# SudeepDasari/visual_foresight

Hardware: AMD Instinct MI355X
Metric: predicted frames/sec (whole node), 200-sample x 13-step x 64x64 CEM (higher is better)
Workload: dtype f32

## Files before the change

visual_foresight_amd/csrc/vf_conv_gsplit.h:

```cpp
#pragma once
#include <hip/hip_runtime.h>
#include "vf_conv_mfma.h"

namespace vf {

__host__ __device__ inline unsigned gs_live_rows(const int img, const int rem, const int yy, const int n_here,
                                                 const int TH, const int TW, const int ty0, const int tx0, const int Hout,
                                                 const int Wout, const int Hin) {
    const int y = ty0 + yy, x = tx0 + rem - yy * TW;
    if (img >= n_here || rem >= TH * TW || y >= Hout || x >= Wout) return 0u;
    unsigned bits = 0u;
    for (int ky = 0; ky < 5; ++ky) bits |= ((unsigned)(y + ky - 2) < (unsigned)Hin ? 1u : 0u) << ky;
    return bits;
}
enum GsRowVariant { GS_ROW_ALL = 0, GS_ROW_FROM1, GS_ROW_TO3, GS_ROW_TO2, GS_ROW_NONE };
__host__ __device__ constexpr int gs_row_variant(const unsigned live4, const int ky) {
    return ky == 0 ? (live4 == 0u ? GS_ROW_NONE : (!(live4 & 1u) ? GS_ROW_FROM1 : GS_ROW_ALL))
                   : (ky == 4 ? (live4 == 0u ? GS_ROW_NONE : (!(live4 & 12u) ? GS_ROW_TO2 : (!(live4 & 8u) ? GS_ROW_TO3 : GS_ROW_ALL)))
                              : GS_ROW_ALL);
}
__host__ __device__ constexpr int gs_row_first(const int v) { return v == GS_ROW_FROM1 ? 1 : 0; }
__host__ __device__ constexpr int gs_row_end(const int v) {
    return v == GS_ROW_NONE ? 0 : (v == GS_ROW_TO3 ? 3 : (v == GS_ROW_TO2 ? 2 : 4));
}
// ... 37 lines not shown
        }
        gbTab[i] = g; gbTab[gbC + i] = b;
    }

    int ab4[MR];
    unsigned live_rows = 0u;
    {
        const int px_per_img = p.TH * p.TW;
        const TileDiv div_rpi(p.RPI), div_tw(p.TW);
#pragma unroll
        for (int m = 0; m < MR; ++m) {
            const int row = m * 32 + n;
            const int img = div_rpi.div(row), rem = row - img * p.RPI;
            const bool ok = img < p.NI && rem < px_per_img;
            const int y = div_tw.div(rem), x = rem - y * p.TW;
            ab4[m] = ((ok ? (img * tile_px + y * LW + x) * KCpad : 0) + kh * 4) >> 2;
            if constexpr (MR == 4) {
                if (p.pad_skip) {
                    const unsigned bits = gs_live_rows(img, rem, y, min(p.NI, p.B - bimg0), p.TH, p.TW, ty0, tx0, p.Hout,
                                                       p.Wout, p.Hin);
#pragma unroll
                    for (int ky = 0; ky < 5; ++ky)
                        if (__builtin_amdgcn_ballot_w64(((bits >> ky) & 1u) != 0u) != 0ull) live_rows |= 1u << (4 * ky + m);
                }
            }
        }
        live_rows = (MR != 4 || !p.pad_skip) ? 0xFFFFFu : (unsigned)__builtin_amdgcn_readfirstlane((int)live_rows);
    }
    f32x16 acc[MR][1];
#pragma unroll
    for (int m = 0; m < MR; ++m)
#pragma unroll
        for (int r = 0; r < 16; ++r) acc[m][0][r] = 0.f;

    const int Ntot = p.ncg * G * 32;
    const int total_chunks = p.seg[0].nchunk + (p.nseg > 1 ? p.seg[1].nchunk : 0);
    const int gtN = total_chunks * 25;
    const unsigned gs_loff = (unsigned)(((kh * Ntot + (cg * G + wave) * 32 + n) * 4) * 4);
    const unsigned gs_wstep_b = (unsigned)(2 * Ntot * 4) * 4u;
    const __amdgpu_buffer_rsrc_t gs_rsrc =
        __builtin_amdgcn_make_buffer_rsrc(const_cast<float *>(p.Wp), 0, 0x7FFFFFFF, 0x00020000);
    f32x4 gsW[4];
    auto gs_loadq = [&](const int q_, const int gt) {
        const unsigned so_ = (unsigned)(min(gt, gtN - 1) * 4 + q_) * gs_wstep_b;
        gsW[q_] = __builtin_bit_cast(f32x4, __builtin_amdgcn_raw_buffer_load_b128(gs_rsrc, gs_loff, so_, 0));
    };
    const int ci0 = p.chunk_begin;
#pragma unroll
    for (int q_ = 0; q_ < 4; ++q_) gs_loadq(q_, ci0 * 25);

    const unsigned magic_px = 0xFFFFFFFFu / (unsigned)tile_px + 1u, magic_lw = 0xFFFFFFFFu / (unsigned)LW + 1u;
    const int q = tid & (q4 - 1), pl = tid >> q4_log2;
    constexpr int ppp = kConvThreads >> q4_log2;
    const int npix = p.NI * tile_px;
    const int y0 = ty0 - 2, x0 = tx0 - 2;
    const int n_here = min(p.NI, p.B - bimg0);
    const bool ni1 = p.NI == 1;
    struct ChunkSrc {
        __amdgpu_buffer_rsrc_t rsrc;
        unsigned cbyte, cstride, img_step;
        int seg, gi;
        bool has_ln, relu;
    };
    auto chunk_src = [&](const int ci) {
        ChunkSrc cs;
        cs.seg = (ci < p.seg[0].nchunk) ? 0 : 1;
// ... 207 lines not shown
```

visual_foresight_amd/csrc/vf_conv_mfma.h:

```cpp
#pragma once
#include <hip/hip_runtime.h>
#include <type_traits>

#ifdef VF_HOST_SELFTEST
#define VF_GLOBAL __device__
#define VF_LAUNCH_BOUNDS(...)
#else
#define VF_GLOBAL __global__
#define VF_LAUNCH_BOUNDS(...) __launch_bounds__(__VA_ARGS__)
#endif

namespace vf {

constexpr int kPollSleep = 16;

#ifdef VF_TILE_STATS
__device__ unsigned long long g_tile_clk[32][8];
#define VF_TS_NOW() (threadIdx.x == 0 ? wall_clock64() : 0ull)
#define VF_TS_ADD(KEY_, SLOT_, DT_) do { if (threadIdx.x == 0) atomicAdd(&g_tile_clk[KEY_][SLOT_], (unsigned long long)(DT_)); } while (0)
#else
#define VF_TS_NOW() 0ull
#define VF_TS_ADD(KEY_, SLOT_, DT_) do { } while (0)
#endif

// ... 78 lines not shown
    int KC;
    int NI, TH, TW, RPI;
    int tilesY, tilesX;
    int ncg;
    int Cout;
    const float *Wp;
    const unsigned short *Wp16;
    const float *bias;
    const float *sbias;
    int sbias_ld;
    float *out;
    float *cstate;
    const float *cstate_in;
    long long cin_bstride;
    long long *stats;
    int stats_nparts;
    int chunks_per_split;
    int n_valid;
    int tile_variant;
    const void *fuse_comp;
    const void *fuse_next;
    int *fuse_ready;
    const int *fuse_status;
    int fuse_view, fuse_nd;
    const int *late_cnt;
    int late_expect, late_mode;
    int *late_status;
    int *cu_state;
    int yield_budget;
    int wt_out;
    const float *cond_bias;
    int chunk_begin;
    int pad_skip;
};

constexpr unsigned kLateSpinLimit = 1u << 26;

constexpr int kYieldSleep = 8;
constexpr int kCtlMyState = 40, kCtlPartnerState = 42;
__device__ __forceinline__ int *ctl_state_word(const int which) {
    extern __shared__ __attribute__((aligned(16))) float smem_all[];
    return *reinterpret_cast<int *const *>(smem_all + which);
}
template <class PT>
__device__ __forceinline__ void cu_publish(const PT &p, const int critical) {
    if (p.cu_state != nullptr && threadIdx.x == 0)
        __hip_atomic_store(ctl_state_word(kCtlMyState), critical, __ATOMIC_RELAXED, __HIP_MEMORY_SCOPE_AGENT);
}
template <class PT>
__device__ __forceinline__ const int *cu_partner_word(const PT &) {
    const unsigned long long a = reinterpret_cast<unsigned long long>(ctl_state_word(kCtlPartnerState));
    const unsigned lo = __builtin_amdgcn_readfirstlane((unsigned)a), hi = __builtin_amdgcn_readfirstlane((unsigned)(a >> 32));
    return reinterpret_cast<const int *>(((unsigned long long)hi << 32) | lo);
}
__device__ __forceinline__ unsigned yield_peek_issue(const int *word) {
    unsigned v;
    asm volatile("s_load_dword %0, %1, 0x0 glc" : "=s"(v) : "s"(word) : "memory");
    return v;
}
__device__ __forceinline__ unsigned yield_peek_wait(unsigned v) {
    asm volatile("s_waitcnt lgkmcnt(0)" : "+s"(v) : : "memory");
    return v;
}
__device__ __forceinline__ void yield_to_partner(const int *word, unsigned seen, int &budget) {
    seen = yield_peek_wait(seen);
    if (seen == 0u || budget <= 0) return;
// ... 369 lines not shown
                __hip_atomic_store(dst + 1, sq, __ATOMIC_RELAXED, __HIP_MEMORY_SCOPE_AGENT);
            } else {
                dst[0] = su; dst[1] = sq;
            }
        };
        if (p.NI == 1) {
            if (tid == 0 && bimg0 < p.B) {
                long long su = 0, sq = 0;
                for (int w = 0; w < 4; ++w) { su += red[2 * w]; sq += red[2 * w + 1]; }
                put(p.stats + ((long long)bimg0 * p.stats_nparts + tile_id * p.ncg + cg) * 2, su, sq);
            }
        } else {
            const int waves_per_img = p.RPI / WROWS;
            if (lane == 0 && (wave % waves_per_img) == 0) {
                const int img = wave / waves_per_img;
                const int b = bimg0 + img;
                if (img < p.NI && b < p.B) {
                    long long su = 0, sq = 0;
                    for (int w = 0; w < waves_per_img; ++w) { su += red[2 * (wave + w)]; sq += red[2 * (wave + w) + 1]; }
                    put(p.stats + ((long long)b * p.stats_nparts + cg) * 2, su, sq);
                }
            }
        }
    }
}

template <class F, int... I>
__device__ __forceinline__ void static_for_impl(F &&f, std::integer_sequence<int, I...>) {
    (f(std::integral_constant<int, I>{}), ...);
}
template <int N, class F>
__device__ __forceinline__ void static_for(F &&f) { static_for_impl(f, std::make_integer_sequence<int, N>{}); }

constexpr int kGsXchFloats = 4 * 4 * 16 * 64;
constexpr int kGsCondFloats = kGsXchFloats + 16 + 25 * 128 + 128;
template <int MR, class PT>
__device__ __forceinline__ void lstm_gsplit_epilogue(const PT &p, f32x16 (&acc)[MR][1], const int bx, const int by,
                                                     float *smem) {
    const int tid = threadIdx.x, lane = tid & 63, wave = tid >> 6;
    const int n = lane & 31, kh = lane >> 5;
    const int cg = by;
    const int tiles_per_img = p.tilesY * p.tilesX;
    int bimg0, ty0, tx0, tile_id;
    if (p.NI == 1) {
        bimg0 = bx / tiles_per_img;
        tile_id = bx % tiles_per_img;
        ty0 = (tile_id / p.tilesX) * p.TH;
        tx0 = (tile_id % p.tilesX) * p.TW;
    } else {
        bimg0 = bx * p.NI;
        tile_id = 0; ty0 = 0; tx0 = 0;
    }
    const int ch = cg * 32 + n;
    float *xch = smem;
    long long *red = reinterpret_cast<long long *>(smem + MR * 4 * 16 * 64);
    const bool wt = p.wt_out != 0;

    const long long img_elems = (long long)p.Hout * p.Wout * p.Cout;
    const TileDiv div_rpi(p.RPI), div_tw(p.TW);
    const int n_here = min(p.NI, p.B - bimg0);
    const unsigned img_bytes = (unsigned)img_elems * 4u;
    const unsigned cin_step = (unsigned)p.cin_bstride * 4u;
    const int span_out = n_here > 0 ? (int)((unsigned)(n_here - 1) * img_bytes + img_bytes) : 0;
    const int span_cin = n_here > 0 ? (int)((unsigned)(n_here - 1) * cin_step + img_bytes) : 0;
    const __amdgpu_buffer_rsrc_t r_cin = __builtin_amdgcn_make_buffer_rsrc(
        const_cast<float *>(p.cstate_in + (long long)bimg0 * p.cin_bstride), 0, span_cin, 0x00020000);
// ... 303 lines not shown
    else if constexpr (EPI == EPI_BIAS_RELU) ts_key = p.KH == 1 ? 17 : (p.seg[0].C == 32 ? 18 : 19);
    else if constexpr (EPI == EPI_CONVT_RELU) ts_key = p.nseg == 1 ? 20 : 21;
    else if constexpr (EPI == EPI_PARTIAL) ts_key = 22;
    else if constexpr (is_top_fused(EPI)) ts_key = 23;
    else if constexpr (EPI == EPI_CONVT_RAW_STATS) ts_key = 24;
    const bool late = p.late_cnt != nullptr;
    ln_table(p, bimg0, lnTab, 0, late ? 1 : 2);
    [[maybe_unused]] const bool yielding = kInLaunch && EPI == EPI_LSTM && (GSPLIT || ROW32) && late &&
                                           p.cu_state != nullptr && p.yield_budget > 0;
    [[maybe_unused]] int ybudget = p.yield_budget;
    [[maybe_unused]] const int *yword = yielding ? cu_partner_word(p) : nullptr;

    const int px_per_img = p.TH * p.TW;
    int abase[MR];
    {
        const TileDiv div_rpi(p.RPI), div_tw(p.TW);
#pragma unroll
        for (int m = 0; m < MR; ++m) {
            const int row = wrow0 + m * 32 + n;
            const int img = div_rpi.div(row), rem = row - img * p.RPI;
            const bool ok = img < p.NI && rem < px_per_img;
            const int y = div_tw.div(rem), x = rem - y * p.TW;
            abase[m] = (ok ? (img * tile_px + y * p.stride * LW + x * p.stride) * KCpad : 0) + kh * 4;
        }
    }

    f32x16 acc[MR][GA];
#pragma unroll
    for (int m = 0; m < MR; ++m)
#pragma unroll
        for (int g = 0; g < GA; ++g)
#pragma unroll
            for (int r = 0; r < 16; ++r) acc[m][g][r] = 0.f;

    const int ntaps = p.KH * p.KW;
    const int Ntot = p.ncg * G * 32;
    const int total_chunks = p.seg[0].nchunk + (p.nseg > 1 ? p.seg[1].nchunk : 0);
    const int ch_begin = bz * p.chunks_per_split;
    const int ch_end = min(ch_begin + p.chunks_per_split, total_chunks);
    const float *wlane = p.Wp + ((long long)kh * Ntot + (cg * G) * 32 + n) * 4;
    const long long wstep = (long long)2 * Ntot * 4;

    const int q4 = KC >> 2;
    const int q4_log2 = 31 - __builtin_clz((unsigned)q4);
    const unsigned magic_px = 0xFFFFFFFFu / (unsigned)tile_px + 1u, magic_lw = 0xFFFFFFFFu / (unsigned)LW + 1u;
    const int items = p.NI * tile_px * q4;

    constexpr bool kGbTab = EPI == EPI_LSTM;
    const int gbC = kGbTab ? ((p.seg[0].C + (p.nseg > 1 ? p.seg[1].C : 0) + 3) & ~3) : 0;
    float *gbTab = lnTab + 4 * p.NI + 16;
    if constexpr (kGbTab) {
        for (int i = tid; i < gbC; i += kConvThreads) {
            const int sgi = i < p.seg[0].C ? 0 : 1;
            const int cc = sgi ? i - p.seg[0].C : i;
            float g = 1.f, b = 0.f;
            if (sgi < p.nseg && cc < p.seg[sgi].C && p.seg[sgi].ln_part) {
                const int m = cc % p.seg[sgi].gamma_mod;
                g = p.seg[sgi].gamma[m]; b = p.seg[sgi].beta[m];
            }
            gbTab[i] = g; gbTab[gbC + i] = b;
        }
    }
    f32x4 *bsm = reinterpret_cast<f32x4 *>(gbTab + 2 * gbC);
    const float *wgate = p.Wp + ((long long)kh * Ntot + (cg * G + (wave & (G - 1))) * 32 + n) * 4;
    const int gt0 = ch_begin * ntaps, gtN = ch_end * ntaps;
    f32x4 breg[4];
#define VF_LOADB(GT_)                                                                           \
    _Pragma("unroll") for (int q = 0; q < 4; ++q)                                               \
        if (q < K8) breg[q] = *reinterpret_cast<const f32x4 *>(wgate + ((long long)(GT_) * K8 + q) * wstep);
#define VF_WRITEB(BUF_)                                                                         \
    _Pragma("unroll") for (int q = 0; q < 4; ++q)                                               \
// ... 562 lines not shown
```

visual_foresight_amd/csrc/vf_engine.hip:

```cpp
#include <hip/hip_runtime.h>

#include <algorithm>
#include <cmath>
#include <cstdio>
#include <cstring>
#include <cstdlib>
#include <string>
#include <vector>

#include <dlfcn.h>
#ifdef VF_HOST_SELFTEST
#include <sys/mman.h>
#endif

#include "../../include/vf_hip.h"
#include "vf_conv_mfma.h"
#include "vf_small_kernels.h"
#include "vf_goal_image.h"
#include "vf_frame_scorer.h"
#include "vf_plan_render.h"
#include "vf_conv_bf16x6.h"
#include "vf_persistent.h"

#ifndef VF_WT_DEFAULT
// ... 315 lines not shown
                                    const size_t unit = ((((size_t)(ci * ntaps + tap) * l.ncg + cgi) * 4 + g) * 3 + pl) * 64 +
                                                        kh * 32 + nn;
                                    out[unit * 8 + j] = pc[pl];
                                }
                            }
    }
    return out;
}

static std::vector<float> pack_bias(const ConvLayer &l, const float *b) {
    const int G = l.G;
    std::vector<float> out((size_t)l.ncg * G * 32, 0.f);
    for (int cgi = 0; cgi < l.ncg; ++cgi)
        for (int g = 0; g < G; ++g)
            for (int nn = 0; nn < 32; ++nn) {
                const int co = cgi * 32 + nn;
                if (co >= l.Cout) continue;
                const int src = l.mode == PACK_LSTM ? g * l.Cout + co : co;
                out[((size_t)cgi * G + g) * 32 + nn] = b[src];
            }
    return out;
}

}

using namespace vf;

struct BatchView {
    float *enc0_o, *enc1_o, *enc2_o, *enc3_o, *enc4_o, *enc5_o, *enc6_o;
    float *enc00_o, *enc7_o;
    float *c_state[7], *h_state[7][2];
    long long *st_enc0, *st_h[7], *st_enc6, *st_enc00, *st_enc7;
    float *sbias, *fc_part, *kern;
    float *cond_bias[7][2];
    float *frames_all, *distrib_all, *states_all;
    double *sums;
    const float *actions;
};

struct LayerW { float *w = nullptr, *b = nullptr; unsigned short *w16 = nullptr; };
struct ViewData {
    LayerW lw[kNumConvLayers];
    float *ln_g[kNumLn] = {nullptr}, *ln_b[kNumLn] = {nullptr};
    float *w_rgb = nullptr, *b_rgb = nullptr, *w_mask = nullptr, *b_mask = nullptr;
    float *w_state = nullptr, *b_state = nullptr, *w_sa = nullptr, *b_fc = nullptr;
    float *w_cond[7] = {nullptr};
    float *ctx_frames = nullptr, *ctx_distrib = nullptr;
};

struct AllocRec { void *p; size_t bytes; };

struct vf_handle {
    vf_config cfg;
    int H, W, T, S, ND, K;
    bool savp = false;
    vf::Savp3 *s3 = nullptr;
    bool cond = false;
    float *cond_bias[7] = {nullptr};
    int Hc, Wc;
    int c_t2 = 64, c_top = 32;
    int ncam = 1, n_draws = 1;
    int ntiles;
    int nblocks;
    std::vector<TensorDesc> table;
    size_t blob_floats = 0;
    bool have_weights = false, have_context = false;
// ... 27 lines not shown
    double *goal_mse = nullptr;

    std::vector<AllocRec> allocs;

    bool dedup = true;
    std::vector<BatchView> shared_views;

    bool persistent = false;
    int n_cu = 256;
    float *actions_buf = nullptr;
    struct SchedCache {
        PhaseDesc *d_phases = nullptr;
        int B = -1, items = 0, counters = 0, phases = 0;
        bool dedup = true;
        int xcd_queues = 0, nq = 1, total_q[kQueues] = {0};
        int options = -1;
        double flops = 0.0;
        size_t lds = 0;
        std::vector<int> types, nitems;
    } sched[2];
    int last_sched = 0;
    size_t sched_capacity = 0, counter_capacity = 0;
    PhaseDesc *stage[kSchedRing] = {nullptr};
    hipEvent_t stage_done[kSchedRing] = {nullptr};
    bool stage_used[kSchedRing] = {false};
    int stage_next = 0;
    int *d_sync = nullptr;
    int xcd_queues = kQueues;
    bool early_start = true;
    bool fuse_top = true;
    bool fuse_pair = true;
    bool wt_publish = VF_WT_DEFAULT != 0;
    bool pad_skip = true;
    int yield_budget = -1;
    bool pair_allowed = true;
    int *d_status = nullptr;
    unsigned long long *d_stats = nullptr;
    bool phase_stats = false;
    int persist_wgs_per_cu = 2;
    size_t max_lds = 0;

    bool cache_shared = true, shared_valid = false;
    int shared_cfg = -1;

    bool profiling = false;
    std::vector<hipEvent_t> ev_pool;
    size_t ev_used = 0;
    double prof_flops = 0.0;

#ifdef VF_HOST_SELFTEST
    char *fake_base = nullptr;
    size_t fake_used = 0, fake_size = 0;
    unsigned long long upload_checksum = 0;
#endif
};

namespace vf {

template <typename T>
static int dev_alloc(vf_handle *h, T **p, size_t n) {
    const size_t bytes = std::max<size_t>(n, 1) * sizeof(T);
    void *q = nullptr;
#ifdef VF_HOST_SELFTEST
    const size_t aligned = (bytes + 255) & ~(size_t)255;
    if (h->fake_used + aligned > h->fake_size) return fail(VF_ERR_NOMEM, "self-test address space exhausted");
    q = h->fake_base + h->fake_used;
// ... 439 lines not shown
        for (int k = 0; k < 7; ++k) VF_ALLOC(h->cond_bias[k], 2 * BV * kCondClasses * 4 * L[k]);
    VF_ALLOC(h->fc_part, BV * h->fc.nsplit * kTaps * h->K);
    VF_ALLOC(h->kern, BV * kTaps * h->K);
    VF_ALLOC(h->frames_all, BV * h->T * H * W * 3);
    VF_ALLOC(h->distrib_all, BV * h->T * H * W * ND);
    VF_ALLOC(h->states_all, BV * h->T * cfg->sdim);
    h->sums_view_stride = (long long)Bc * ND * h->nblocks * 2;
    h->sums_step_stride = h->sums_view_stride * NV;
    VF_ALLOC(h->sums, (size_t)h->T * h->sums_step_stride);
    VF_ALLOC(h->goal_mse, BV * h->T);
    VF_ALLOC(h->actions_buf, (size_t)Bc * h->T * cfg->adim);
    h->sched_capacity = ((size_t)h->S * 32 + 8) * NV;
    h->counter_capacity = ((size_t)h->S * 32 + 8) * ((size_t)Bc + 1) * NV;
    VF_ALLOC(h->sched[0].d_phases, h->sched_capacity);
    VF_ALLOC(h->sched[1].d_phases, h->sched_capacity);
    VF_ALLOC(h->d_sync, kSyncHead + h->counter_capacity);
    VF_ALLOC(h->d_status, 1);
    VF_ALLOC(h->d_stats, h->sched_capacity * 2);
    for (int i = 0; i < NV; ++i) {
        BatchView sv;
        memset(&sv, 0, sizeof(sv));
        VF_ALLOC(sv.enc0_o, (size_t)H2 * W2 * 32);
        VF_ALLOC(sv.enc1_o, (size_t)H4 * W4 * L[1]);
        VF_ALLOC(sv.enc2_o, (size_t)H8 * W8 * L[3]);
        VF_ALLOC(sv.enc3_o, (size_t)H8 * W8 * L[3]);
        VF_ALLOC(sv.enc4_o, (size_t)H4 * W4 * L[4]);
        VF_ALLOC(sv.enc5_o, (size_t)H2 * W2 * h->c_t2);
        for (int k = 0; k < 7; ++k) {
            const size_t per = (size_t)lh[k] * lw[k] * L[k];
            VF_ALLOC(sv.c_state[k], per);
            VF_ALLOC(sv.h_state[k][0], per);
            VF_ALLOC(sv.h_state[k][1], per);
            VF_ALLOC(sv.st_h[k], (size_t)h->st_rows[k] * 2);
        }
        VF_ALLOC(sv.st_enc0, (size_t)h->enc0.stats_nparts * 2);
        if (h->savp) {
            VF_ALLOC(sv.enc00_o, (size_t)Hc * Wc * kEnc00Ch);
            VF_ALLOC(sv.st_enc00, (size_t)h->enc00.stats_nparts * 2);
        }
        VF_ALLOC(sv.sbias, (size_t)L[3]);
        if (h->cond)
            for (int k = 0; k < 7; ++k) {
                VF_ALLOC(sv.cond_bias[k][0], (size_t)2 * kCondClasses * 4 * L[k]);
                sv.cond_bias[k][1] = sv.cond_bias[k][0] + (size_t)kCondClasses * 4 * L[k];
            }
        h->shared_views.push_back(sv);
    }
#undef VF_ALLOC
    return VF_OK;
}

extern "C" {

int vf_create(const vf_config *cfg, vf_handle **out) {
    vf_handle *made = nullptr;
    VF_API_TRY
    if (!out) return fail(VF_ERR_INVALID, "null out pointer");
    *out = nullptr;
    int rc = validate(cfg);
    if (rc) return rc;
#ifndef VF_HOST_SELFTEST
    VF_HIP_CHECK(hipSetDevice(cfg->device));
#endif
    vf_handle *h = new vf_handle();
    made = h;
    h->cfg = *cfg;
    if (const char *e = getenv("VF_PAD_SKIP")) h->pad_skip = atoi(e) != 0;
    h->ncam = std::max(1, cfg->ncam);
    h->n_draws = std::max(1, cfg->n_draws);
    h->cfg.ncam = h->ncam; h->cfg.n_draws = h->n_draws;
    h->H = cfg->height; h->W = cfg->width; h->ND = cfg->ndesig; h->K = cfg->num_masks;
    h->T = cfg->sequence_length - cfg->n_context;
    h->S = h->T + cfg->n_context - 1;
    h->table = tensor_table(*cfg);
    h->blob_floats = h->table.back().offset + h->table.back().size();
    h->savp = cfg->arch == 1 || cfg->arch == 2;
    h->cond = cfg->arch == 2;
    h->Hc = h->savp ? h->H / 2 : h->H; h->Wc = h->savp ? h->W / 2 : h->W;
    const int H = h->H, W = h->W;
    h->ntiles = ((H + kCompTile - 1) / kCompTile) * ((W + kCompTile - 1) / kCompTile);
    h->nblocks = sum_blocks(H, W);
#ifdef VF_HOST_SELFTEST
    h->fake_size = (size_t)1 << 40;
    void *base = mmap(nullptr, h->fake_size, PROT_NONE, MAP_PRIVATE | MAP_ANONYMOUS | MAP_NORESERVE, -1, 0);
    if (base == MAP_FAILED) { delete h; return fail(VF_ERR_NOMEM, "self-test address reservation failed"); }
    h->fake_base = static_cast<char *>(base);
#endif

    rc = cfg->arch == 3 ? s3_create(h) : cdna_create(h);
    if (rc) { vf_destroy(h); return rc; }
    VF_INJECT(3);
#ifndef VF_HOST_SELFTEST
    if (hipMemset(h->d_sync, 0, kSyncHead * sizeof(int)) != hipSuccess || hipMemset(h->d_status, 0, sizeof(int)) != hipSuccess) {
        vf_destroy(h);
        return fail(VF_ERR_HIP, "hipMemset of the scheduler words failed");
    }
    for (int i = 0; i < kSchedRing; ++i) {
        void *q = nullptr;
        if (hipHostMalloc(&q, h->sched_capacity * sizeof(PhaseDesc), hipHostMallocDefault) != hipSuccess ||
            hipEventCreateWithFlags(&h->stage_done[i], hipEventDisableTiming) != hipSuccess) {
// ... 208 lines not shown
    v.enc6_o = h->enc6_o + b * Hc * Wc * h->c_top;
    for (int k = 0; k < 7; ++k) {
        const size_t per = (size_t)lh[k] * lw[k] * L[k];
        v.c_state[k] = h->c_state[k] + b * per;
        v.h_state[k][0] = h->h_state[k][0] + b * per;
        v.h_state[k][1] = h->h_state[k][1] + b * per;
        v.st_h[k] = h->st_h[k] + b * h->st_rows[k] * 2;
    }
    v.st_enc0 = h->st_enc0 + b * h->enc0.stats_nparts * 2;
    v.st_enc6 = h->st_enc6 + b * h->convt3.stats_nparts * 2;
    v.sbias = h->sbias + b * L[3];
    if (h->cond)
        for (int k = 0; k < 7; ++k)
            for (int par = 0; par < 2; ++par)
                v.cond_bias[k][par] = h->cond_bias[k] + ((size_t)par * c.max_batch * h->ncam + b) * kCondClasses * 4 * L[k];
    v.fc_part = h->fc_part + b * h->fc.nsplit * kTaps * h->K;
    v.kern = h->kern + b * kTaps * h->K;
    v.frames_all = h->frames_all + b * T * H * W * 3;
    v.distrib_all = h->distrib_all + b * T * H * W * ND;
    v.states_all = h->states_all + b * T * c.sdim;
    v.sums = h->sums + (long long)view * h->sums_view_stride + (size_t)b0 * ND * h->nblocks * 2;
    v.actions = d_actions + (size_t)b0 * T * c.adim;
    return v;
}

static const int kSkipped = 1 << 30;

#ifndef VF_HOST_SELFTEST
struct LaunchSink {
    vf_handle *h;
    hipStream_t st;
    static int skipped() { return VF_OK; }

    int conv(int type, const ConvLayer &l, const ConvParams &p, std::initializer_list<int>) {
        switch (type) {
            case PH_LSTM: {
                if (!h->profiling) return launch_lstm(l, p, st);
                while (h->ev_pool.size() < h->ev_used + 2) {
                    hipEvent_t e;
                    VF_HIP_CHECK(hipEventCreate(&e));
                    h->ev_pool.push_back(e);
                }
                VF_HIP_CHECK(hipEventRecord(h->ev_pool[h->ev_used], st));
                int r = launch_lstm(l, p, st);
                VF_HIP_CHECK(hipEventRecord(h->ev_pool[h->ev_used + 1], st));
                h->ev_used += 2;
                h->prof_flops += 2.0 * (p.B * l.Hout * l.Wout * 25.0 - (p.pad_skip ? 5.0 * gs_pad_skipped_pairs(l, p.B) : 0.0)) *
                                 (l.segC[0] + l.segC[1]) * 4.0 * l.Cout;
                return r;
            }
            case PH_CONV_RELU: return launch_conv_t<1, EPI_BIAS_RELU>(l, p, st);
            case PH_CONV_RAW:
                if (l.tile == TILE_FIRST_VALU) {
                    const dim3 grid(p.B * l.tilesY * l.tilesX);
                    if (l.Cout == 16) hipLaunchKernelGGL(conv_first_kernel<16>, grid, dim3(kConvThreads), l.lds_bytes, st, p);
                    else hipLaunchKernelGGL(conv_first_kernel<32>, grid, dim3(kConvThreads), l.lds_bytes, st, p);
                    VF_HIP_CHECK(hipGetLastError());
                    return VF_OK;
                }
                return launch_conv_t<1, EPI_RAW_STATS>(l, p, st);
            case PH_CONVT_RELU: return launch_conv_t<4, EPI_CONVT_RELU>(l, p, st);
            case PH_CONVT_RAW: return launch_conv_t<4, EPI_CONVT_RAW_STATS>(l, p, st);
            case PH_CONV_RAW3: return l.mrep == 2 ? launch_conv_m<1, EPI_RAW, 2>(l, p, st) : launch_conv_m<1, EPI_RAW, 1>(l, p, st);
            case PH_CONV_RAW3G2: return l.mrep == 2 ? launch_conv_m<2, EPI_RAW, 2>(l, p, st) : launch_conv_m<2, EPI_RAW, 1>(l, p, st);
            case PH_CONV_RAW3G4: return launch_conv_m<4, EPI_RAW, 1>(l, p, st);
            case PH_GATES_RAW: {
                const int tiles = l.NI == 1 ? p.B * l.tilesY * l.tilesX : (p.B + l.NI - 1) / l.NI;
                hipLaunchKernelGGL(conv_gates_raw_kernel, dim3(tiles, l.ncg), dim3(kConvThreads), l.lds_bytes, st, p);
                VF_HIP_CHECK(hipGetLastError());
                return VF_OK;
            }
            default: return launch_conv_t<1, EPI_PARTIAL>(l, p, st);
        }
    }
    int ew(const EwParams &p, int , std::initializer_list<int>) {
        const int items = p.spi > 0 ? (p.B + p.spi - 1) / p.spi : p.B * p.gx;
        const size_t lds = ew_lds_bytes(p.op, h->ND);
        switch (h->ND) {
            case 1: hipLaunchKernelGGL(ew_kernel<1>, dim3(items), dim3(kConvThreads), lds, st, p); break;
            case 2: hipLaunchKernelGGL(ew_kernel<2>, dim3(items), dim3(kConvThreads), lds, st, p); break;
            case 3: hipLaunchKernelGGL(ew_kernel<3>, dim3(items), dim3(kConvThreads), lds, st, p); break;
            default: hipLaunchKernelGGL(ew_kernel<4>, dim3(items), dim3(kConvThreads), lds, st, p); break;
        }
        VF_HIP_CHECK(hipGetLastError());
        return VF_OK;
    }
    int lstm(const ConvLayer &l, const ConvParams &p, int , int , int  = -1) { return conv(PH_LSTM, l, p, {}); }
    int cond(const CondParams &p, std::initializer_list<int>) {
        hipLaunchKernelGGL(cond_bias_kernel, dim3((p.B + kCondPerItem - 1) / kCondPerItem), dim3(256), 0, st, p);
        VF_HIP_CHECK(hipGetLastError());
        return VF_OK;
    }
    int conv_late(int type, const ConvLayer &l, const ConvParams &p, int , int , int  = -1) { return conv(type, l, p, {}); }
    static bool pair_capable() { return false; }
    static const ConvLayer &fc_plan(const vf_handle *h) { return h->fc; }
    int conv_pair(const ConvLayer &, const ConvParams &, const ConvLayer &, const ConvParams &, std::initializer_list<int>) {
        return VF_ERR_INVALID;
    }
    int sa(const SaParams &p, std::initializer_list<int>) {
        hipLaunchKernelGGL(sa_kernel, dim3(p.B), dim3(64), 0, st, p);
        return VF_OK;
    }
    int fin(const FinParams &p, std::initializer_list<int>) {
// ... 235 lines not shown
        s.ln_inv_n = (float)(1.0 / (double)count); s.gamma = g; s.beta = b; s.gamma_mod = gmod; s.relu = relu;
        return s;
    };
#define VF_EMIT(var, expr)                 \
    const int var = (expr);                \
    if (Sink::failed(var)) return var;
#define VF_EMIT_SH(var, shared, expr) VF_EMIT(var, ((shared) && skip_shared) ? Sink::skipped() : (expr))

    int last = -1;
    int u_cond_next[7] = {-1, -1, -1, -1, -1, -1, -1};
    int u_prev[7] = {-1, -1, -1, -1, -1, -1, -1};
    for (int s = 0; s < h->S; ++s) {
        const int cur = s & 1, nxt = cur ^ 1;
        const bool produce = s >= nc - 1;
        const int t_out = s - (nc - 1);
        const bool enc0_sh = enc_shared(s), enc_sh = core_shared(s), all_sh = all_shared(s);
        const BatchView &E0 = enc0_sh ? sh : v;
        const BatchView &E = enc_sh ? sh : v;
        const BatchView &D = all_sh ? sh : v;
        const int BE0 = enc0_sh ? 1 : B, BE = enc_sh ? 1 : B, BD = all_sh ? 1 : B;
        auto bs = [](bool shared, long long per) { return shared ? 0LL : per; };

        SaParams sp; memset(&sp, 0, sizeof(sp));
        if (s < nc - 1) { sp.action = h->ctx_actions + (size_t)s * c.adim; sp.action_bstride = 0; }
        else { sp.action = v.actions + (size_t)(s - (nc - 1)) * c.adim; sp.action_bstride = (long long)T * c.adim; }
        if (s < nc) { sp.state = h->ctx_states + (size_t)s * c.sdim; sp.state_bstride = 0; }
        else { sp.state = v.states_all + (size_t)(s - nc) * c.sdim; sp.state_bstride = (long long)T * c.sdim; }
        sp.adim = c.adim; sp.sdim = c.sdim; sp.B = BD;
        sp.w_state = vd.w_state; sp.b_state = vd.b_state; sp.w_sa = vd.w_sa; sp.n_out = L[3];
        sp.state_out = produce ? v.states_all + (size_t)t_out * c.sdim : nullptr;
        sp.state_out_bstride = (long long)T * c.sdim;
        sp.sbias = D.sbias;
        VF_EMIT_SH(u_sa, all_sh, sink.sa(sp, {last}))

        int u_cond[7];
        for (int k = 0; k < 7; ++k) u_cond[k] = u_cond_next[k];
        auto emit_cond = [&](const int sc, const int u_state, int (&out)[7]) -> int {
            for (int k = 0; k < 7; ++k) out[k] = -1;
            if (!h->cond || sc >= h->S) return VF_OK;
            const float *act, *sta; long long act_bs, sta_bs;
            if (sc < nc - 1) { act = h->ctx_actions + (size_t)sc * c.adim; act_bs = 0; }
            else { act = v.actions + (size_t)(sc - (nc - 1)) * c.adim; act_bs = (long long)T * c.adim; }
            if (sc < nc) { sta = h->ctx_states + (size_t)sc * c.sdim; sta_bs = 0; }
            else { sta = v.states_all + (size_t)(sc - nc) * c.sdim; sta_bs = (long long)T * c.sdim; }
            for (int k = 0; k < 7; ++k) {
                const bool shd = lstm_shared(k, sc);
                CondParams cq; memset(&cq, 0, sizeof(cq));
                cq.action = act; cq.action_bstride = act_bs;
                cq.state = sta; cq.state_bstride = sta_bs;
                cq.adim = c.adim; cq.sdim = c.sdim; cq.B = shd ? 1 : B;
                cq.w = vd.w_cond[k]; cq.C4 = 4 * L[k];
                cq.out = (shd ? sh : v).cond_bias[k][sc & 1];
                VF_EMIT_SH(u_ck, shd, sink.cond(cq, {u_state}))
                out[k] = u_ck;
            }
            return VF_OK;
        };
        if (s == 0) {
            const int rc0 = emit_cond(0, -1, u_cond);
            if (Sink::failed(rc0)) return rc0;
        }

        const float *frame_in; long long frame_bs;
        if (s < nc) { frame_in = vd.ctx_frames + (size_t)s * H * W * 3; frame_bs = 0; }
        else { frame_in = v.frames_all + (size_t)(s - nc) * H * W * 3; frame_bs = (long long)T * H * W * 3; }

// ... 8 lines not shown
            enc00_n = normed(E0.enc00_o, bs(enc0_sh, (long long)Hc * Wc * kEnc00Ch), E0.st_enc00, h->enc00.stats_nparts,
                             h->enc00.stats_nparts, enc0_sh, (long long)Hc * Wc * kEnc00Ch, vd.ln_g[9], vd.ln_b[9],
                             kEnc00Ch, 1);
        }
        p = params(h->enc0, BE0, h->savp ? enc00_n : plain(frame_in, frame_bs), nullptr);
        p.out = E0.enc0_o; p.stats = E0.st_enc0;
        VF_EMIT_SH(u_enc0, enc0_sh, sink.conv(PH_CONV_RAW, h->enc0, p, {u_enc00}))

        SegArg enc0_n = normed(E0.enc0_o, bs(enc0_sh, (long long)H2 * W2 * 32), E0.st_enc0, h->enc0.stats_nparts,
                               h->enc0.stats_nparts, enc0_sh, (long long)H2 * W2 * 32, vd.ln_g[0], vd.ln_b[0], 32, 1);
        auto h_normed = [&](int k) {
            const bool shd = lstm_shared(k, s);
            const BatchView &O = shd ? sh : v;
            const long long per = (long long)lh[k] * lw[k] * L[k];
            return normed(O.h_state[k][nxt], bs(shd, per), O.st_h[k], lstm_plan(k, shd ? 1 : B).stats_nparts,
                          h->st_rows[k], shd, per, vd.ln_g[k + 1], vd.ln_b[k + 1], L[k], 0);
        };
        auto lstm_params = [&](int k, const SegArg &x) {
            const bool out_sh = lstm_shared(k, s), in_sh = lstm_shared(k, s - 1);
            const BatchView &O = out_sh ? sh : v, &I = in_sh ? sh : v;
            const long long per = (long long)lh[k] * lw[k] * L[k];
            SegArg hs = plain(I.h_state[k][cur], bs(in_sh, per));
            ConvParams q = params(lstm_plan(k, out_sh ? 1 : B), out_sh ? 1 : B, hs, &x);
            q.out = O.h_state[k][nxt]; q.cstate = O.c_state[k]; q.stats = O.st_h[k];
            q.stats_nparts = h->st_rows[k];
            q.cstate_in = I.c_state[k]; q.cin_bstride = bs(in_sh, per);
            if (h->cond) q.cond_bias = O.cond_bias[k][s & 1];
#ifdef VF_DEBUG_KNOBS
            static const bool no_rec = getenv("VF_TIMING_NO_RECURRENT") && atoi(getenv("VF_TIMING_NO_RECURRENT"));
            if (no_rec) { q.seg[0].nchunk = 0; q.chunks_per_split = q.seg[1].nchunk; }
#endif
            return q;
        };
        VF_EMIT_SH(u_l1, lstm_shared(0, s), sink.lstm(lstm_plan(0, lstm_shared(0, s) ? 1 : B), lstm_params(0, enc0_n), u_prev[0], u_enc0, u_cond[0]))
        VF_EMIT_SH(u_l2, lstm_shared(1, s), sink.lstm(lstm_plan(1, lstm_shared(1, s) ? 1 : B), lstm_params(1, h_normed(0)), u_prev[1], u_l1, u_cond[1]))

        p = params(h->enc1, BE, h_normed(1), nullptr);
        p.out = E.enc1_o;
        VF_EMIT_SH(u_enc1, enc_sh, sink.conv(PH_CONV_RELU, h->enc1, p, {u_l2}))

        VF_EMIT_SH(u_l3, lstm_shared(2, s), sink.lstm(lstm_plan(2, lstm_shared(2, s) ? 1 : B),
                                lstm_params(2, plain(E.enc1_o, bs(enc_sh, (long long)H4 * W4 * L[1]))), u_prev[2], u_enc1, u_cond[2]))
        VF_EMIT_SH(u_l4, lstm_shared(3, s), sink.lstm(lstm_plan(3, lstm_shared(3, s) ? 1 : B), lstm_params(3, h_normed(2)), u_prev[3], u_l3, u_cond[3]))

        const ConvLayer &enc2_l = light_plan(h->enc2, h->enc2_one, BE);
        const ConvLayer &enc3_l = light_plan(h->enc3, h->enc3_one, BD);
        p = params(enc2_l, BE, h_normed(3), nullptr);
        p.out = E.enc2_o;
        ConvParams p3 = params(enc3_l, BD, plain(E.enc2_o, bs(enc_sh, (long long)H8 * W8 * L[3])), nullptr);
        p3.out = D.enc3_o; p3.sbias = D.sbias; p3.sbias_ld = L[3];
        int u_enc3 = -1;
        const bool pair_ok = Sink::pair_capable() && h->fuse_pair && enc_sh == all_sh && BE == BD;
        if (pair_ok && !ScheduleSink::pairable(enc2_l, enc3_l) && ScheduleSink::pairable(enc2_l, h->enc3)) {
            p3 = params(h->enc3, BD, plain(E.enc2_o, bs(enc_sh, (long long)H8 * W8 * L[3])), nullptr);
            p3.out = D.enc3_o; p3.sbias = D.sbias; p3.sbias_ld = L[3];
            VF_EMIT_SH(u_pair, enc_sh, sink.conv_pair(enc2_l, p, h->enc3, p3, {u_l4, u_sa}))
            u_enc3 = u_pair;
        } else if (pair_ok && ScheduleSink::pairable(enc2_l, enc3_l)) {
            VF_EMIT_SH(u_pair, enc_sh, sink.conv_pair(enc2_l, p, enc3_l, p3, {u_l4, u_sa}))
            u_enc3 = u_pair;
        } else {
            VF_EMIT_SH(u_enc2, enc_sh, sink.conv(PH_CONV_RELU, enc2_l, p, {u_l4}))
            VF_EMIT_SH(u_enc3_, all_sh, sink.conv(PH_CONV_RELU, enc3_l, p3, {u_enc2, u_sa}))
            u_enc3 = u_enc3_;
        }

        VF_EMIT_SH(u_l5, lstm_shared(4, s), sink.lstm(lstm_plan(4, lstm_shared(4, s) ? 1 : B),
                                lstm_params(4, plain(D.enc3_o, bs(all_sh, (long long)H8 * W8 * L[3]))), u_prev[4], u_enc3, u_cond[4]))
        SegArg h5n = h_normed(4);

        const ConvLayer &convt1_l = light_plan(h->convt1, h->convt1_one, BD);
        p = params(convt1_l, BD, h5n, nullptr);
        p.out = D.enc4_o;
        {
            const int rcn = emit_cond(s + 1, u_sa, u_cond_next);
            if (Sink::failed(rcn)) return rcn;
        }
        VF_EMIT_SH(u_t1, all_sh, sink.conv(PH_CONVT_RELU, convt1_l, p, {u_l5}))
        VF_EMIT_SH(u_l6, lstm_shared(5, s), sink.lstm(lstm_plan(5, lstm_shared(5, s) ? 1 : B),
                                lstm_params(5, plain(D.enc4_o, bs(all_sh, (long long)H4 * W4 * L[4]))), u_prev[5], u_t1, u_cond[5]))

        int u_fin = -1, u_fc = -1;
        if (produce) {
            SegArg flat = h5n;
            const ConvLayer &fc_l = Sink::fc_plan(h);
            p = params(fc_l, B, flat, nullptr);
            p.out = v.fc_part;
            VF_EMIT(u_fc_, sink.conv(PH_FC_PARTIAL, fc_l, p, {u_l5}))
            u_fc = u_fc_;
        }

        SegArg enc1_s = plain(E.enc1_o, bs(enc_sh, (long long)H4 * W4 * L[1])), h6n = h_normed(5);
        p = params(h->convt2, BD, enc1_s, &h6n);
        p.out = D.enc5_o;
        VF_EMIT_SH(u_t2, all_sh, sink.conv_late(PH_CONVT_RELU, h->convt2, p, u_enc1, u_l6))
        VF_EMIT_SH(u_l7, lstm_shared(6, s), sink.lstm(lstm_plan(6, lstm_shared(6, s) ? 1 : B),
                                lstm_params(6, plain(D.enc5_o, bs(all_sh, (long long)H2 * W2 * h->c_t2))), u_prev[6], u_t2, u_cond[6]))
        last = u_l7;
        {
            const int now[7] = {u_l1, u_l2, u_l3, u_l4, u_l5, u_l6, u_l7};
            for (int k = 0; k < 7; ++k) u_prev[k] = now[k];
        }
        if (produce) {
            FinParams fp;
            fp.partial = v.fc_part; fp.nsplit = h->fc.nsplit; fp.B = B; fp.K = h->K;
            fp.bias = vd.b_fc; fp.kern = v.kern;
            u_fin = sink.fin(fp, {u_fc});
            if (Sink::failed(u_fin)) return u_fin;
        }

        if (produce) {
            SegArg h7n = h_normed(6);
            p = params(h->convt3, B, enc0_n, &h7n);
            p.out = v.enc6_o; p.stats = v.st_enc6;
            const ConvLayer *top_l = &h->convt3;
            int top_early = u_enc0, top_late = u_l7;
            if (h->savp) {
                SegArg enc6_n = normed(v.enc6_o, (long long)Hc * Wc * 32, v.st_enc6, h->convt3.stats_nparts,
                                       h->convt3.stats_nparts, false, (long long)Hc * Wc * 32, vd.ln_g[8], vd.ln_b[8], 32, 1);
                VF_EMIT(u_t3, sink.conv_late(PH_CONVT_RAW, h->convt3, p, u_enc0, u_l7))
                p = params(h->convt4, B, enc00_n, &enc6_n);
                p.out = v.enc7_o; p.stats = v.st_enc7;
                top_l = &h->convt4; top_early = u_enc00; top_late = u_t3;
            }

            CompositeParams cp; memset(&cp, 0, sizeof(cp));
            cp.B = B; cp.H = H; cp.W = W; cp.ND = ND; cp.K = h->K;
            if (h->savp) {
                cp.enc6 = v.enc7_o; cp.ln_part = v.st_enc7; cp.ln_nparts = h->convt4.stats_nparts;
                cp.gamma = vd.ln_g[10]; cp.beta = vd.ln_b[10];
// ... 177 lines not shown
        ticket += P.n_items;
        if (P.ndep < 0 || P.ndep > kMaxDeps) return fail(VF_ERR_INVALID, "bad dependency count");
        for (int d = 0; d < P.ndep; ++d) {
            bool found = false;
            for (size_t j = 0; j < i && !found; ++j) found = bs.phases[j].cnt_base == P.dep[d].cnt_base;
            if (!found) return fail(VF_ERR_INVALID, "phase " + std::to_string(i) + " depends on a later phase");
            if (P.dep[d].expect <= 0) return fail(VF_ERR_INVALID, "non-positive expected count");
        }
        if (P.has_late) {
            bool found = false;
            for (size_t j = 0; j < i && !found; ++j) found = bs.phases[j].cnt_base == P.late.cnt_base;
            if (!found || !(ph_is_conv(P.type) || P.type == PH_TOP_FUSED) || P.late.expect <= 0)
                return fail(VF_ERR_INVALID, "phase " + std::to_string(i) + ": bad late dependency");
        }
        const int ncnt = P.whole ? 1 : (P.type == PH_TOP_FUSED ? 2 * P.B : P.B);
        if (P.cnt_base < 0 || P.cnt_base + ncnt > bs.counters) return fail(VF_ERR_INVALID, "counter out of range");
        bool ok = true;
        if (P.type == PH_CONV_PAIR) {
            const ConvParams &c2 = P.conv2;
            ok = ok && P.conv.ncg == 1 && c2.ncg == 2 && c2.KC == 32 && c2.nseg == 1 && c2.seg[0].nchunk == 2;
            ok = ok && in_allocs(h, c2.Wp, (size_t)2 * 4 * 2 * 64 * 4 * 4) && in_allocs(h, c2.bias, 64 * 4);
            ok = ok && in_allocs(h, c2.out, (size_t)P.B * c2.Hout * c2.Wout * c2.Cout * 4);
            ok = ok && in_allocs(h, c2.sbias, c2.sbias ? (size_t)((P.B - 1) * c2.sbias_ld + c2.Cout) * 4 : 0);
        }
        if (P.type <= PH_FC_PARTIAL || ph_is_conv(P.type) || P.type == PH_TOP_FUSED || P.type == PH_CONV_PAIR) {
            const ConvParams &c = P.conv;
            for (int s = 0; s < c.nseg; ++s) {
                const long long span = (long long)(P.B - 1) * c.seg[s].bstride + (long long)c.Hin * c.Win * c.seg[s].C;
                ok = ok && in_allocs(h, c.seg[s].ptr, (size_t)span * 4);
                ok = ok && in_allocs(h, c.seg[s].ln_part, c.seg[s].ln_part ? (size_t)((P.B - 1) * c.seg[s].ln_bstride + c.seg[s].ln_nparts * 2) * 8 : 0);
            }
            ok = ok && in_allocs(h, c.Wp, 16) && in_allocs(h, c.bias, 4) && in_allocs(h, c.out, 4);
            ok = ok && in_allocs(h, c.cstate, 4) && in_allocs(h, c.cstate_in, 4) && in_allocs(h, c.stats, 8);
        }
        if (P.conv.wt_out != 0) {
            const bool lstm_vec = P.type == PH_LSTM &&
                                  (P.tile == TILE_LSTM_GS128 || P.tile == TILE_LSTM_GS64 || P.tile == TILE_LSTM_ROW32);
            const bool light_vec = P.type >= PH_CONV_RELU && P.type <= PH_CONVT_RAW && P.conv.Cout % 4 == 0 &&
                                   ((P.tile == TILE_CONV && P.mrep == 1) ||
                                    (P.tile == TILE_FIRST_VALU && P.type == PH_CONV_RAW && (P.conv.Cout == 16 || P.conv.Cout == 32)));
            const bool raw3_vec = (P.type == PH_CONV_RAW3 || P.type == PH_CONV_RAW3G2 || P.type == PH_CONV_RAW3G4) &&
                                  P.tile == TILE_CONV && (P.mrep == 1 || P.mrep == 2) && P.conv.Cout % 4 == 0;
            if (!(lstm_vec || light_vec || raw3_vec || P.type == PH_GATES_RAW || P.type == PH_TOP_FUSED))
                return fail(VF_ERR_INVALID, "phase " + std::to_string(i) + ": write-through publish on a tile with plain stores");
        }
        if (P.type == PH_EW && P.ew.wt != 0) {
            const int op = P.ew.op;
            const bool vec = op == EW_INORM || op == EW_INCELL || op == EW_UPSAMPLE ||
                             (op == EW_TOP3 && P.ew.top.H % 4 == 0 && P.ew.top.W % 16 == 0);
            if (!vec) return fail(VF_ERR_INVALID, "phase " + std::to_string(i) + ": write-through publish on an item with plain stores");
        }
        if (P.type == PH_TOP_FUSED && (P.aux_base != P.cnt_base + P.B || P.aux_base + P.B > bs.counters))
            return fail(VF_ERR_INVALID, "fused phase: bad auxiliary counters");
        if (P.type <= PH_FC_PARTIAL || ph_is_conv(P.type)) {
        } else if (P.type == PH_EW) {
            const EwParams &e = P.ew;
            if (e.op == EW_INORM || e.op == EW_INCELL) {
                const NormParams &q = e.norm;
                const size_t hw = (size_t)q.H * q.W, ctot = (size_t)(e.op == EW_INCELL ? 4 : 1) * q.C;
                ok = ok && in_allocs(h, q.in, ((size_t)(P.B - 1) * q.in_bs + hw * ctot) * 4);
                const size_t co = q.split > 0 ? (size_t)q.split : (size_t)q.C;
                ok = ok && in_allocs(h, q.out, ((size_t)(P.B - 1) * q.out_bs + hw * co) * 4);
                ok = ok && (q.split == 0 || (in_allocs(h, q.out2, ((size_t)(P.B - 1) * q.out_bs + hw * co) * 4) && q.C == 2 * q.split));
                ok = ok && in_allocs(h, q.cond, q.cond ? ((size_t)(P.B - 1) * q.cond_bs + 25 * ctot) * 4 : 0);
                ok = ok && in_allocs(h, q.g0, ctot * 4) && in_allocs(h, q.b0, ctot * 4) && q.C % q.cpi == 0 && e.gx == q.C / q.cpi;
                ok = ok && in_allocs(h, q.tab, q.tab ? (size_t)P.B * q.C * 2 * 4 : 0);
// ... 782 lines not shown
```

Before: 42660.

## Share recurrent gate partial sums across samples when hidden state is still shared

When an LSTM layer's previous-step hidden state was shared across all samples (batch-1) but the current step is per-sample, the recurrent half of the gate convolution is computed once for a single image into a scratch buffer. The per-sample LSTM kernels then start their accumulators from that buffer via acc_init and only process the input-channel chunks (chunk_begin offset). This removes redundant recurrent-weight convolution work across the batch. The cost is an extra launch and a dependency edge, plus a scratch buffer and extra per-lane loads at accumulator init.

```diff
diff --git a/visual_foresight_amd/csrc/vf_conv_gsplit.h b/visual_foresight_amd/csrc/vf_conv_gsplit.h
--- a/visual_foresight_amd/csrc/vf_conv_gsplit.h
+++ b/visual_foresight_amd/csrc/vf_conv_gsplit.h
@@ -93,6 +93,9 @@
     for (int m = 0; m < MR; ++m)
 #pragma unroll
         for (int r = 0; r < 16; ++r) acc[m][0][r] = 0.f;
+    if constexpr (!RAW) {
+        if (p.acc_init != nullptr) gs_acc_init<MR>(p, acc, cg, ty0, tx0);
+    }
 
     const int Ntot = p.ncg * G * 32;
     const int total_chunks = p.seg[0].nchunk + (p.nseg > 1 ? p.seg[1].nchunk : 0);
diff --git a/visual_foresight_amd/csrc/vf_conv_mfma.h b/visual_foresight_amd/csrc/vf_conv_mfma.h
--- a/visual_foresight_amd/csrc/vf_conv_mfma.h
+++ b/visual_foresight_amd/csrc/vf_conv_mfma.h
@@ -134,6 +134,7 @@
     const float *cond_bias;
     int chunk_begin;
     int pad_skip;
+    const float *acc_init;
 };
 
 constexpr unsigned kLateSpinLimit = 1u << 26;
@@ -569,6 +570,30 @@
 template <int N, class F>
 __device__ __forceinline__ void static_for(F &&f) { static_for_impl(f, std::make_integer_sequence<int, N>{}); }
 
+template <int MR, class PT>
+__device__ __forceinline__ void gs_acc_init(const PT &p, f32x16 (&acc)[MR][1], const int cg, const int ty0, const int tx0) {
+    const int lane = threadIdx.x & 63, wave = threadIdx.x >> 6;
+    const int n = lane & 31, kh = lane >> 5;
+    const unsigned px_b = (unsigned)(4 * p.Cout) * 4u;
+    const unsigned col_b = (unsigned)(wave * p.Cout + cg * 32 + n) * 4u;
+    const __amdgpu_buffer_rsrc_t rs = __builtin_amdgcn_make_buffer_rsrc(
+        const_cast<float *>(p.acc_init), 0, (int)((unsigned)(p.Hout * p.Wout) * px_b), 0x00020000);
+    const TileDiv div_tw(p.TW);
+#pragma unroll
+    for (int m = 0; m < MR; ++m)
+#pragma unroll
+        for (int j = 0; j < 4; ++j) {
+            const int rem = m * 32 + 8 * j + 4 * kh;
+            const int yy = div_tw.div(rem);
+            const int y = ty0 + yy, x = tx0 + rem - yy * p.TW;
+            const bool ok = rem < p.TH * p.TW && y < p.Hout && x < p.Wout;
+            const unsigned off = (ok ? (unsigned)(y * p.Wout + x) * px_b : 0u) + col_b;
+#pragma unroll
+            for (int i = 0; i < 4; ++i)
+                acc[m][0][4 * j + i] = __builtin_bit_cast(float, __builtin_amdgcn_raw_buffer_load_b32(rs, off, (unsigned)i * px_b, 0));
+        }
+}
+
 constexpr int kGsXchFloats = 4 * 4 * 16 * 64;
 constexpr int kGsCondFloats = kGsXchFloats + 16 + 25 * 128 + 128;
 template <int MR, class PT>
@@ -938,11 +963,14 @@
         for (int g = 0; g < GA; ++g)
 #pragma unroll
             for (int r = 0; r < 16; ++r) acc[m][g][r] = 0.f;
+    if constexpr (GSPLIT) {
+        if (p.acc_init != nullptr) gs_acc_init<MR>(p, acc, cg, ty0, tx0);
+    }
 
     const int ntaps = p.KH * p.KW;
     const int Ntot = p.ncg * G * 32;
     const int total_chunks = p.seg[0].nchunk + (p.nseg > 1 ? p.seg[1].nchunk : 0);
-    const int ch_begin = bz * p.chunks_per_split;
+    const int ch_begin = bz * p.chunks_per_split + (GSPLIT ? p.chunk_begin : 0);
     const int ch_end = min(ch_begin + p.chunks_per_split, total_chunks);
     const float *wlane = p.Wp + ((long long)kh * Ntot + (cg * G) * 32 + n) * 4;
     const long long wstep = (long long)2 * Ntot * 4;
diff --git a/visual_foresight_amd/csrc/vf_engine.hip b/visual_foresight_amd/csrc/vf_engine.hip
--- a/visual_foresight_amd/csrc/vf_engine.hip
+++ b/visual_foresight_amd/csrc/vf_engine.hip
@@ -371,6 +371,7 @@
     float *c_state[7], *h_state[7][2];
     long long *st_enc0, *st_h[7], *st_enc6, *st_enc00, *st_enc7;
     float *sbias, *fc_part, *kern;
+    float *rec_part[7];
     float *cond_bias[7][2];
     float *frames_all, *distrib_all, *states_all;
     double *sums;
@@ -464,6 +465,7 @@
     bool fuse_pair = true;
     bool wt_publish = VF_WT_DEFAULT != 0;
     bool pad_skip = true;
+    bool share_recurrent = true;
     int yield_budget = -1;
     bool pair_allowed = true;
     int *d_status = nullptr;
@@ -969,6 +971,7 @@
             VF_ALLOC(sv.h_state[k][0], per);
             VF_ALLOC(sv.h_state[k][1], per);
             VF_ALLOC(sv.st_h[k], (size_t)h->st_rows[k] * 2);
+            if (h->share_recurrent && h->lstm[k].tile == TILE_LSTM_GS128) VF_ALLOC(sv.rec_part[k], 4 * per);
         }
         VF_ALLOC(sv.st_enc0, (size_t)h->enc0.stats_nparts * 2);
         if (h->savp) {
@@ -1003,6 +1006,7 @@
     made = h;
     h->cfg = *cfg;
     if (const char *e = getenv("VF_PAD_SKIP")) h->pad_skip = atoi(e) != 0;
+    if (const char *e = getenv("VF_SHARE_RECURRENT")) h->share_recurrent = atoi(e) != 0;
     h->ncam = std::max(1, cfg->ncam);
     h->n_draws = std::max(1, cfg->n_draws);
     h->cfg.ncam = h->ncam; h->cfg.n_draws = h->n_draws;
@@ -1277,23 +1281,25 @@
     hipStream_t st;
     static int skipped() { return VF_OK; }
 
+    template <class F>
+    int profiled_lstm(const ConvLayer &l, const ConvParams &p, F launch) {
+        if (!h->profiling) return launch();
+        while (h->ev_pool.size() < h->ev_used + 2) {
+            hipEvent_t e;
+            VF_HIP_CHECK(hipEventCreate(&e));
+            h->ev_pool.push_back(e);
+        }
+        VF_HIP_CHECK(hipEventRecord(h->ev_pool[h->ev_used], st));
+        int r = launch();
+        VF_HIP_CHECK(hipEventRecord(h->ev_pool[h->ev_used + 1], st));
+        h->ev_used += 2;
+        h->prof_flops += 2.0 * (p.B * l.Hout * l.Wout * 25.0 - (p.pad_skip ? 5.0 * gs_pad_skipped_pairs(l, p.B) : 0.0)) *
+                         (l.segC[0] + (l.nseg > 1 ? l.segC[1] : 0) - p.chunk_begin * l.KC) * 4.0 * l.Cout;
+        return r;
+    }
     int conv(int type, const ConvLayer &l, const ConvParams &p, std::initializer_list<int>) {
         switch (type) {
-            case PH_LSTM: {
-                if (!h->profiling) return launch_lstm(l, p, st);
-                while (h->ev_pool.size() < h->ev_used + 2) {
-                    hipEvent_t e;
-                    VF_HIP_CHECK(hipEventCreate(&e));
-                    h->ev_pool.push_back(e);
-                }
-                VF_HIP_CHECK(hipEventRecord(h->ev_pool[h->ev_used], st));
-                int r = launch_lstm(l, p, st);
-                VF_HIP_CHECK(hipEventRecord(h->ev_pool[h->ev_used + 1], st));
-                h->ev_used += 2;
-                h->prof_flops += 2.0 * (p.B * l.Hout * l.Wout * 25.0 - (p.pad_skip ? 5.0 * gs_pad_skipped_pairs(l, p.B) : 0.0)) *
-                                 (l.segC[0] + l.segC[1]) * 4.0 * l.Cout;
-                return r;
-            }
+            case PH_LSTM: return profiled_lstm(l, p, [&] { return launch_lstm(l, p, st); });
             case PH_CONV_RELU: return launch_conv_t<1, EPI_BIAS_RELU>(l, p, st);
             case PH_CONV_RAW:
                 if (l.tile == TILE_FIRST_VALU) {
@@ -1310,10 +1316,13 @@
             case PH_CONV_RAW3G2: return l.mrep == 2 ? launch_conv_m<2, EPI_RAW, 2>(l, p, st) : launch_conv_m<2, EPI_RAW, 1>(l, p, st);
             case PH_CONV_RAW3G4: return launch_conv_m<4, EPI_RAW, 1>(l, p, st);
             case PH_GATES_RAW: {
-                const int tiles = l.NI == 1 ? p.B * l.tilesY * l.tilesX : (p.B + l.NI - 1) / l.NI;
-                hipLaunchKernelGGL(conv_gates_raw_kernel, dim3(tiles, l.ncg), dim3(kConvThreads), l.lds_bytes, st, p);
-                VF_HIP_CHECK(hipGetLastError());
-                return VF_OK;
+                auto launch = [&]() -> int {
+                    const int tiles = l.NI == 1 ? p.B * l.tilesY * l.tilesX : (p.B + l.NI - 1) / l.NI;
+                    hipLaunchKernelGGL(conv_gates_raw_kernel, dim3(tiles, l.ncg), dim3(kConvThreads), l.lds_bytes, st, p);
+                    VF_HIP_CHECK(hipGetLastError());
+                    return VF_OK;
+                };
+                return h->cfg.arch == 3 ? launch() : profiled_lstm(l, p, launch);
             }
             default: return launch_conv_t<1, EPI_PARTIAL>(l, p, st);
         }
@@ -1615,6 +1624,23 @@
         sp.state_out_bstride = (long long)T * c.sdim;
         sp.sbias = D.sbias;
         VF_EMIT_SH(u_sa, all_sh, sink.sa(sp, {last}))
+
+        bool rec_sh[7];
+        int u_part[7];
+        for (int k = 0; k < 7; ++k) {
+            rec_sh[k] = false; u_part[k] = -1;
+            if (!sh.rec_part[k] || nc < 2 || s < 1 || !lstm_shared(k, s - 1) || lstm_shared(k, s)) continue;
+            const ConvLayer &cl = lstm_plan(k, B);
+            ConvLayer pl = h->lstm[k];
+            if (pl.tile != TILE_LSTM_GS128 || (cl.tile != TILE_LSTM_GS128 && cl.tile != TILE_LSTM_GS64) || cl.NI != 1 ||
+                cl.TW % 4 || cl.Wout % 4 || cl.KC != pl.KC || cl.nchunk[0] != pl.nchunk[0] || pl.segC[0] % pl.KC)
+                continue;
+            pl.nseg = 1; pl.segC[1] = 0; pl.nchunk[1] = 0; pl.chunks_per_split = pl.nchunk[0];
+            ConvParams q = params(pl, 1, plain(sh.h_state[k][cur], 0), nullptr);
+            q.out = sh.rec_part[k];
+            VF_EMIT_SH(u_p, true, sink.conv(PH_GATES_RAW, pl, q, {u_prev[k]}))
+            rec_sh[k] = true; u_part[k] = u_p;
+        }
 
         int u_cond[7];
         for (int k = 0; k < 7; ++k) u_cond[k] = u_cond_next[k];
@@ -1689,16 +1715,24 @@
 #endif
             return q;
         };
-        VF_EMIT_SH(u_l1, lstm_shared(0, s), sink.lstm(lstm_plan(0, lstm_shared(0, s) ? 1 : B), lstm_params(0, enc0_n), u_prev[0], u_enc0, u_cond[0]))
-        VF_EMIT_SH(u_l2, lstm_shared(1, s), sink.lstm(lstm_plan(1, lstm_shared(1, s) ? 1 : B), lstm_params(1, h_normed(0)), u_prev[1], u_l1, u_cond[1]))
+        auto emit_lstm = [&](int k, const SegArg &x, int u_x) -> int {
+            const bool shd = lstm_shared(k, s);
+            if (shd && skip_shared) return Sink::skipped();
+            const ConvLayer &l = lstm_plan(k, shd ? 1 : B);
+            ConvParams q = lstm_params(k, x);
+            if (!rec_sh[k]) return sink.lstm(l, q, u_prev[k], u_x, u_cond[k]);
+            q.chunk_begin = q.seg[0].nchunk; q.acc_init = sh.rec_part[k];
+            return sink.conv(PH_LSTM, l, q, {u_part[k], u_x, u_cond[k]});
+        };
+        VF_EMIT(u_l1, emit_lstm(0, enc0_n, u_enc0))
+        VF_EMIT(u_l2, emit_lstm(1, h_normed(0), u_l1))
 
         p = params(h->enc1, BE, h_normed(1), nullptr);
         p.out = E.enc1_o;
         VF_EMIT_SH(u_enc1, enc_sh, sink.conv(PH_CONV_RELU, h->enc1, p, {u_l2}))
 
-        VF_EMIT_SH(u_l3, lstm_shared(2, s), sink.lstm(lstm_plan(2, lstm_shared(2, s) ? 1 : B),
-                                lstm_params(2, plain(E.enc1_o, bs(enc_sh, (long long)H4 * W4 * L[1]))), u_prev[2], u_enc1, u_cond[2]))
-        VF_EMIT_SH(u_l4, lstm_shared(3, s), sink.lstm(lstm_plan(3, lstm_shared(3, s) ? 1 : B), lstm_params(3, h_normed(2)), u_prev[3], u_l3, u_cond[3]))
+        VF_EMIT(u_l3, emit_lstm(2, plain(E.enc1_o, bs(enc_sh, (long long)H4 * W4 * L[1])), u_enc1))
+        VF_EMIT(u_l4, emit_lstm(3, h_normed(2), u_l3))
 
         const ConvLayer &enc2_l = light_plan(h->enc2, h->enc2_one, BE);
         const ConvLayer &enc3_l = light_plan(h->enc3, h->enc3_one, BD);
@@ -1722,8 +1756,7 @@
             u_enc3 = u_enc3_;
         }
 
-        VF_EMIT_SH(u_l5, lstm_shared(4, s), sink.lstm(lstm_plan(4, lstm_shared(4, s) ? 1 : B),
-                                lstm_params(4, plain(D.enc3_o, bs(all_sh, (long long)H8 * W8 * L[3]))), u_prev[4], u_enc3, u_cond[4]))
+        VF_EMIT(u_l5, emit_lstm(4, plain(D.enc3_o, bs(all_sh, (long long)H8 * W8 * L[3])), u_enc3))
         SegArg h5n = h_normed(4);
 
         const ConvLayer &convt1_l = light_plan(h->convt1, h->convt1_one, BD);
@@ -1734,8 +1767,7 @@
             if (Sink::failed(rcn)) return rcn;
         }
         VF_EMIT_SH(u_t1, all_sh, sink.conv(PH_CONVT_RELU, convt1_l, p, {u_l5}))
-        VF_EMIT_SH(u_l6, lstm_shared(5, s), sink.lstm(lstm_plan(5, lstm_shared(5, s) ? 1 : B),
-                                lstm_params(5, plain(D.enc4_o, bs(all_sh, (long long)H4 * W4 * L[4]))), u_prev[5], u_t1, u_cond[5]))
+        VF_EMIT(u_l6, emit_lstm(5, plain(D.enc4_o, bs(all_sh, (long long)H4 * W4 * L[4])), u_t1))
 
         int u_fin = -1, u_fc = -1;
         if (produce) {
@@ -1751,8 +1783,7 @@
         p = params(h->convt2, BD, enc1_s, &h6n);
         p.out = D.enc5_o;
         VF_EMIT_SH(u_t2, all_sh, sink.conv_late(PH_CONVT_RELU, h->convt2, p, u_enc1, u_l6))
-        VF_EMIT_SH(u_l7, lstm_shared(6, s), sink.lstm(lstm_plan(6, lstm_shared(6, s) ? 1 : B),
-                                lstm_params(6, plain(D.enc5_o, bs(all_sh, (long long)H2 * W2 * h->c_t2))), u_prev[6], u_t2, u_cond[6]))
+        VF_EMIT(u_l7, emit_lstm(6, plain(D.enc5_o, bs(all_sh, (long long)H2 * W2 * h->c_t2)), u_t2))
         last = u_l7;
         {
             const int now[7] = {u_l1, u_l2, u_l3, u_l4, u_l5, u_l6, u_l7};
@@ -1996,6 +2027,14 @@
             }
             ok = ok && in_allocs(h, c.Wp, 16) && in_allocs(h, c.bias, 4) && in_allocs(h, c.out, 4);
             ok = ok && in_allocs(h, c.cstate, 4) && in_allocs(h, c.cstate_in, 4) && in_allocs(h, c.stats, 8);
+            const size_t gates_bytes = (size_t)c.Hout * c.Wout * 4 * c.Cout * 4;
+            if (P.type == PH_GATES_RAW) ok = ok && in_allocs(h, c.out, (size_t)P.B * gates_bytes);
+            if (c.chunk_begin != 0)
+                ok = ok && (P.type == PH_GATES_RAW ||
+                            (P.type == PH_LSTM && (P.tile == TILE_LSTM_GS128 || P.tile == TILE_LSTM_GS64)));
+            if (c.acc_init)
+                ok = ok && in_allocs(h, c.acc_init, gates_bytes) && P.type == PH_LSTM && P.NI == 1 && !P.has_late &&
+                     (P.tile == TILE_LSTM_GS128 || P.tile == TILE_LSTM_GS64) && c.chunk_begin == c.seg[0].nchunk;
         }
         if (P.conv.wt_out != 0) {
             const bool lstm_vec = P.type == PH_LSTM &&
```

Result: faster. 44250, median of 6 (+3.7%).
